# Xharlie/pointnerf

Hardware: AMD Instinct MI355X
Metric: rays/sec (render+bwd) NeRF-synth lego 800^2, K=8, 128 samp/ray (higher is better)
Workload: dtype f32 in / out / accumulate; forward GEMM operands as 2 x f16 planes (22-bit) on the f16 MFMA, 3 products per multiply-add; input-gradient GEMMs: f16 leading product + e4m3 cross terms (csrc/mixq.h), 2 product equivalents; weight-gradient GEMM operands as one f16 plane each

## Files before the change

### pointnerf_amd/csrc/backward.hip

```cpp
#include "mixq.h"

namespace {
constexpr int WG_CHUNKS = 256;
constexpr size_t PARTIAL_FLOATS = (size_t)WG_CHUNKS * PN_H * PN_IN1P;

struct BwdArgs {
    pnerf_camera cam;
    const float *params;
    const float4 *packed;
    const float *raydir;
    const int *pidx, *valid_list, *counters;
    const int *cls_list, *cls_info;
    int cls;
    int SR, K, TS;
    long long cap_samples;
    const float *decoded, *weight, *grad_decoded;
    PnSaved sv;
    const float *emb;
    float *gparams;
    float *g_emb, *g_conf, *g_dir, *g_color;
    const float *conf, *zo_gs;
    float zo_eps;
};
struct BwdXArgs : BwdArgs {
    const float *xyz, *sample_loc;
    float *g_xyz;
};
template <bool XYZG> struct BwdArgsOf { using T = BwdArgs; };
template <> struct BwdArgsOf<true> { using T = BwdXArgs; };

__global__ __launch_bounds__(256) void k_grad_max(const int *__restrict__ list, const int *__restrict__ counters, long long cap, const float *__restrict__ gd,
                                                  unsigned *__restrict__ gscale) {
    __shared__ unsigned red[4];
    const long long Ns = counters[0] < cap ? counters[0] : cap;
    float m = 0.f;
    for (long long vs = (long long)blockIdx.x * 256 + threadIdx.x; vs < Ns; vs += (long long)gridDim.x * 256) {
        const float4 g = *reinterpret_cast<const float4 *>(gd + (long long)list[vs] * 4);
        m = fmaxf(m, fmaxf(fmaxf(fabsf(g.x), fabsf(g.y)), fmaxf(fabsf(g.z), fabsf(g.w))));
    }
#pragma unroll
    for (int off = 32; off > 0; off >>= 1) m = fmaxf(m, __shfl_xor(m, off, 64));
    if ((threadIdx.x & 63) == 0) red[threadIdx.x >> 6] = __float_as_uint(m);
    __syncthreads();
    if (threadIdx.x == 0) {
        unsigned r = red[0];
        for (int i = 1; i < 4; ++i) r = red[i] > r ? red[i] : r;
        if (r != 0u && r < 0x7f800000u) atomicMax(gscale, r);
    }
}
__device__ __forceinline__ void pn_scale_from_bits(unsigned mb, float &S, float &invS) {
    const int e = (int)((mb >> 23) & 0xffu);
    int se = (e == 0 || e == 255) ? 127 : 127 + 4 - (e - 127);
    se = se < 2 ? 2 : (se > 252 ? 252 : se);
    S = __uint_as_float((unsigned)se << 23);
    invS = __uint_as_float((unsigned)(254 - se) << 23);
}
static_assert(PN_CTILE == PN_TILE, "one row-scale record layout for both tile kernels");
constexpr int PN_RSC_BYTES = PN_TILE * 16 + PN_TILE * 2;
__device__ __forceinline__ void pn_sample_scale(const float4 g, float S, float invS, float &Si, float &invSi) {
    const unsigned mb = __float_as_uint(fmaxf(fmaxf(fabsf(g.x), fabsf(g.y)), fmaxf(fabsf(g.z), fabsf(g.w))));
    Si = S; invSi = invS;
    if (mb >= 0x00800000u && mb < 0x7f800000u) {
        pn_scale_from_bits(mb, Si, invSi);
        if (Si < S) { Si = S; invSi = invS; }
    }
}
struct PnRowScale {
    float *p;
    __device__ __forceinline__ void set(int r, float Si, float invSi, float S, float w = 0.f) const {
        const float f = S * invSi;
        *reinterpret_cast<float4 *>(p + 4 * r) = make_float4(Si, invSi, f, w * Si);
        reinterpret_cast<_Float16 *>(p + 4 * PN_TILE)[r] = (_Float16)f;
    }
    __device__ __forceinline__ float S(int r) const { return p[4 * r]; }
    __device__ __forceinline__ float inv(int r) const { return p[4 * r + 1]; }
    __device__ __forceinline__ float to_call(int r) const { return p[4 * r + 2]; }
    __device__ __forceinline__ float wS(int r) const { return p[4 * r + 3]; }
    __device__ __forceinline__ const char *h8(int rg) const { return reinterpret_cast<const char *>(p + 4 * PN_TILE) + rg * 16; }
};
template <int NF, int XRS = PN_XRS>
__device__ __forceinline__ void pn_copy_out_kmajor_hs(const char *X, const PnRowScale &rs, uint4 *__restrict__ dst, long long rg0, int tid) {
    const int lane = tid & 63, wave = tid >> 6;
    const int blk = ((lane >> 2) & 3) * XRS + ((lane >> 4) * 16 + (lane & 3) * 4) * 2;
#pragma unroll
    for (int i = 0; i < 2; ++i) {
        const int rg = wave * 2 + i;
        const char *src = X + rg * 8 * XRS + blk;
        uint4 *d = dst + (rg0 + rg) * NF;
        const uint4 fq = *reinterpret_cast<const uint4 *>(rs.h8(rg));
        const pn_h4 flo = __builtin_bit_cast(pn_h4, make_uint2(fq.x, fq.y)), fhi = __builtin_bit_cast(pn_h4, make_uint2(fq.z, fq.w));
        uint2 lo[(NF + 63) / 64], hi[(NF + 63) / 64];
#pragma unroll
        for (int j = 0; j < (NF + 63) / 64; ++j) { lo[j] = pn_lds_read_tr16(src + j * 128); hi[j] = pn_lds_read_tr16(src + 4 * XRS + j * 128); }
#pragma unroll
        for (int j = 0; j < (NF + 63) / 64; ++j) {
            const int f = lane + 64 * j;
            if (f < NF) {
                const uint2 a = __builtin_bit_cast(uint2, __builtin_bit_cast(pn_h4, lo[j]) * flo), b = __builtin_bit_cast(uint2, __builtin_bit_cast(pn_h4, hi[j]) * fhi);
                pn_f4 t = {__uint_as_float(a.x), __uint_as_float(a.y), __uint_as_float(b.x), __uint_as_float(b.y)};
                PN_STREAM_STORE(t, reinterpret_cast<pn_f4 *>(d + f));
            }
        }
    }
}

constexpr int CB_XRS = 2 * PN_HC + 16, CB_XPL = PN_CTILE * CB_XRS, CB_XBYTES = 2 * CB_XPL;
constexpr int CB_DRAW = CB_XBYTES, CB_GACC = CB_DRAW + PN_CTILE * 4 * 4, CB_W4 = CB_GACC + 6 * PN_HC * 4, CB_RSC = CB_W4 + 3 * PN_HC * 4, CB_BYTES = CB_RSC + PN_RSC_BYTES;
static_assert(3 * CB_BYTES <= 160 * 1024, "three colour workgroups must fit the 160 KB LDS");

__device__ __forceinline__ void cb_epilogue(const f32x16 (&acc)[2][2], unsigned mw, char *X, int wave, int lane) {
#pragma unroll
    for (int rb = 0; rb < 2; ++rb)
#pragma unroll
        for (int g = 0; g < 4; ++g) {
            const int f0 = pn_d_feat(wave, g, lane), row = 32 * rb + (lane & 31), e = rb * 16 + g * 4;
            float v[4];
#pragma unroll
            for (int i = 0; i < 4; ++i) v[i] = acc[0][rb][4 * g + i] * ((int)(mw << (e + i)) < 0 ? 0.01f : 1.f);
            pn_x_store4<true, CB_XRS, CB_XPL>(X, row, f0, v[0], v[1], v[2], v[3]);
        }
}
__device__ __forceinline__ void cb_bias_sums(const char *X, const PnRowScale &rs, int tid, float *__restrict__ gsum) {
    const int c0 = 8 * (tid & 15), r0 = 4 * (tid >> 4);
    float gb[8] = {0.f, 0.f, 0.f, 0.f, 0.f, 0.f, 0.f, 0.f};
#pragma unroll
    for (int rr = 0; rr < 4; ++rr) {
        const uint4 h = *reinterpret_cast<const uint4 *>(X + (r0 + rr) * CB_XRS + c0 * 2);
        const uint4 m = *reinterpret_cast<const uint4 *>(X + CB_XPL + (r0 + rr) * CB_XRS + c0 * 2);
        const float f = rs.to_call(r0 + rr);
        gb[0] = pn_fma2_lo(h.x, m.x, f, gb[0]); gb[1] = pn_fma2_hi(h.x, m.x, f, gb[1]);
        gb[2] = pn_fma2_lo(h.y, m.y, f, gb[2]); gb[3] = pn_fma2_hi(h.y, m.y, f, gb[3]);
        gb[4] = pn_fma2_lo(h.z, m.z, f, gb[4]); gb[5] = pn_fma2_hi(h.z, m.z, f, gb[5]);
        gb[6] = pn_fma2_lo(h.w, m.w, f, gb[6]); gb[7] = pn_fma2_hi(h.w, m.w, f, gb[7]);
    }
#pragma unroll
    for (int i = 0; i < 8; ++i) atomicAdd(gsum + c0 + i, gb[i]);
}

template <bool WG2>
__global__ __launch_bounds__(256, 3) void k_color_backward(BwdArgs a) {
    extern __shared__ __attribute__((aligned(16))) char smem_cb[];
    char *X = smem_cb;
    float *draw = reinterpret_cast<float *>(smem_cb + CB_DRAW);
    const PnRowScale rs{reinterpret_cast<float *>(smem_cb + CB_RSC)};
    const int Ns = a.counters[0] < a.cap_samples ? a.counters[0] : (int)a.cap_samples;
    const float *P = a.params;
    const char *img = reinterpret_cast<const char *>(a.packed);
    float S, invS;
    pn_scale_from_bits(a.sv.gscale[0], S, invS);
    if (blockIdx.x == 0 && threadIdx.x == 0) a.sv.cls_info[PN_CI_CTILES] = (Ns + PN_CTILE - 1) / PN_CTILE;
    float *gacc = reinterpret_cast<float *>(smem_cb + CB_GACC);
    for (int i = threadIdx.x; i < 6 * PN_HC; i += 256) gacc[i] = 0.f;
    float gb4x = 0.f, gb4y = 0.f, gb4z = 0.f;
    auto row_sample = [&](long long t) -> long long {
        const long long vs = t * PN_CTILE + threadIdx.x;
        return (threadIdx.x < PN_CTILE && vs < Ns) ? (long long)a.valid_list[vs] : -1;
    };
    float po[3] = {0.f, 0.f, 0.f}, pg[3] = {0.f, 0.f, 0.f}, pgs = 0.f;
    auto row_values = [&](long long si) {
        if (si >= 0) {
            const float *o = a.decoded + si * 4, *g = a.grad_decoded + si * 4;
            po[0] = o[1]; po[1] = o[2]; po[2] = o[3]; pgs = g[0]; pg[0] = g[1]; pg[1] = g[2]; pg[2] = g[3];
        }
    };
    long long si_cur = row_sample(blockIdx.x);
    row_values(si_cur);
    float *w4s = reinterpret_cast<float *>(smem_cb + CB_W4);
    for (int i = threadIdx.x; i < 3 * PN_HC; i += 256) w4s[i] = P[PO_WC4 + i];

    f32x16 acc[2][2];
    for (long long tile = blockIdx.x; tile * PN_CTILE < Ns; tile += gridDim.x) {
        int tid = threadIdx.x;
        asm volatile("" : "+v"(tid));
        const int lane = tid & 63, wave = __builtin_amdgcn_readfirstlane(tid >> 6);
        const long long grow0 = tile * PN_CTILE;
        PN_LDS_BARRIER();
        if (tid < PN_CTILE) {
            float d0 = 0.f, d1 = 0.f, d2 = 0.f, Si = S, invSi = invS;
            if (si_cur >= 0) {
                pn_sample_scale(make_float4(pgs, pg[0], pg[1], pg[2]), S, invS, Si, invSi);
                const float s0 = (po[0] + 0.001f) / 1.002f, s1 = (po[1] + 0.001f) / 1.002f, s2 = (po[2] + 0.001f) / 1.002f;
                d0 = pg[0] * 1.002f * s0 * (1.f - s0); d1 = pg[1] * 1.002f * s1 * (1.f - s1); d2 = pg[2] * 1.002f * s2 * (1.f - s2);
            }
            *reinterpret_cast<float4 *>(draw + tid * 4) = make_float4(d0, d1, d2, Si);
            rs.set(tid, Si, invSi, S);
            gb4x += d0; gb4y += d1; gb4z += d2;
        }
        const long long si_next = row_sample(tile + gridDim.x);
        PN_LDS_BARRIER();
        {
            const int c4 = tid & 31, rg = tid >> 5;
            float4 c3v[8];
            float w4[3][4], gw4[3][4], gb3[4] = {0.f, 0.f, 0.f, 0.f};
#pragma unroll
            for (int k = 0; k < 3; ++k) {
                const float4 w = *reinterpret_cast<const float4 *>(w4s + k * PN_HC + 4 * c4);
                w4[k][0] = w.x; w4[k][1] = w.y; w4[k][2] = w.z; w4[k][3] = w.w;
#pragma unroll
                for (int i = 0; i < 4; ++i) gw4[k][i] = 0.f;
            }
#pragma unroll
            for (int rr = 0; rr < 8; ++rr) c3v[rr] = *reinterpret_cast<const float4 *>(a.sv.c3 + (grow0 + 8 * rg + rr) * PN_HC + 4 * c4);
#pragma unroll
            for (int rr = 0; rr < 8; ++rr) {
                const int row = 8 * rg + rr;
                const float4 d = *reinterpret_cast<const float4 *>(draw + row * 4);
                const float c[4] = {c3v[rr].x, c3v[rr].y, c3v[rr].z, c3v[rr].w};
                float u[4];
#pragma unroll
                for (int i = 0; i < 4; ++i) {
                    u[i] = (d.x * w4[0][i] + d.y * w4[1][i] + d.z * w4[2][i]) * pn_lrelu_grad(c[i]);
                    gw4[0][i] += d.x * c[i]; gw4[1][i] += d.y * c[i]; gw4[2][i] += d.z * c[i];
                    gb3[i] += u[i];
                }
                pn_x_store4<true, CB_XRS, CB_XPL>(X, row, 4 * c4, u[0] * d.w, u[1] * d.w, u[2] * d.w, u[3] * d.w);
            }
#pragma unroll
            for (int i = 0; i < 4; ++i) {
#pragma unroll
                for (int k = 0; k < 3; ++k) atomicAdd(gacc + k * PN_HC + 4 * c4 + i, gw4[k][i]);
                atomicAdd(gacc + 3 * PN_HC + 4 * c4 + i, gb3[i]);
            }
        }
        PnGemmW<8, 4, 1, 4, 3> WD3;
        WD3.prefetch(reinterpret_cast<const uint4 *>(img + PKH_DC3), wave, lane);
        PN_LDS_BARRIER();
        pn_copy_out_kmajor_hs<PN_HC, CB_XRS>(X, rs, a.sv.dc3k, tile * 8, tid);
        if (WG2) pn_copy_out_kmajor_hs<PN_HC, CB_XRS>(X + CB_XPL, rs, a.sv.dc3m, tile * 8, tid);
        const unsigned mw2 = a.sv.cmask[(tile * 2 + 1) * 256 + tid], mw1 = a.sv.cmask[(tile * 2 + 0) * 256 + tid];
        pn_acc_zero(acc);
        pn_gemm_f16x3_run<8, 4, 1, 4, 3, CB_XRS, CB_XPL>(X, WD3, lane, acc);
        row_values(si_next);
        si_cur = si_next;
        PN_LDS_BARRIER();
        cb_epilogue(acc, mw2, X, wave, lane);
        PnGemmW<8, 4, 1, 4, 3> WD2;
        WD2.prefetch(reinterpret_cast<const uint4 *>(img + PKH_DC2), wave, lane);
        PN_LDS_BARRIER();
        cb_bias_sums(X, rs, tid, gacc + 4 * PN_HC);
        pn_copy_out_kmajor_hs<PN_HC, CB_XRS>(X, rs, a.sv.dc2k, tile * 8, tid);
        if (WG2) pn_copy_out_kmajor_hs<PN_HC, CB_XRS>(X + CB_XPL, rs, a.sv.dc2m, tile * 8, tid);
        pn_acc_zero(acc);
        pn_gemm_f16x3_run<8, 4, 1, 4, 3, CB_XRS, CB_XPL>(X, WD2, lane, acc);
        PN_LDS_BARRIER();
        cb_epilogue(acc, mw1, X, wave, lane);
        PnGemmW<8, 8, 2, 1, 3> WD1;
        WD1.prefetch(reinterpret_cast<const uint4 *>(img + PKH_DC1), 2 * wave, lane);
        PN_LDS_BARRIER();
        cb_bias_sums(X, rs, tid, gacc + 5 * PN_HC);
        pn_copy_out_kmajor_hs<PN_HC, CB_XRS>(X, rs, a.sv.dc1k, tile * 8, tid);
        if (WG2) pn_copy_out_kmajor_hs<PN_HC, CB_XRS>(X + CB_XPL, rs, a.sv.dc1m, tile * 8, tid);
        pn_acc_zero(acc);
        pn_gemm_f16x3_run<8, 8, 2, 1, 3, CB_XRS, CB_XPL>(X, WD1, lane, acc);
#pragma unroll
        for (int fb = 0; fb < 2; ++fb)
#pragma unroll
            for (int rb = 0; rb < 2; ++rb) {
                const float ri = rs.inv(32 * rb + (lane & 31));
#pragma unroll
                for (int g = 0; g < 4; ++g) {
                    pn_f4 t = {acc[fb][rb][4 * g] * ri, acc[fb][rb][4 * g + 1] * ri, acc[fb][rb][4 * g + 2] * ri, acc[fb][rb][4 * g + 3] * ri};
                    PN_REG_STORE(t, reinterpret_cast<pn_f4 *>(a.sv.dfs + (grow0 + 32 * rb + (lane & 31)) * PN_H + pn_d_feat(2 * wave + fb, g, lane)));
                }
            }
    }
    PN_LDS_BARRIER();
    {
        const int tid = threadIdx.x;
        for (int i = tid; i < 3 * PN_HC; i += 256) atomicAdd(&a.gparams[PO_WC4 + i], gacc[i]);
        if (tid < PN_HC) {
            atomicAdd(&a.gparams[PO_BC3 + tid], gacc[3 * PN_HC + tid]);
            atomicAdd(&a.gparams[PO_BC2 + tid], gacc[4 * PN_HC + tid] * invS);
            atomicAdd(&a.gparams[PO_BC1 + tid], gacc[5 * PN_HC + tid] * invS);
        }
        if (tid < PN_CTILE) {
#pragma unroll
            for (int off = 32; off > 0; off >>= 1) { gb4x += __shfl_xor(gb4x, off, 64); gb4y += __shfl_xor(gb4y, off, 64); gb4z += __shfl_xor(gb4z, off, 64); }
            if (tid == 0) { atomicAdd(&a.gparams[PO_BC4], gb4x); atomicAdd(&a.gparams[PO_BC4 + 1], gb4y); atomicAdd(&a.gparams[PO_BC4 + 2], gb4z); }
        }
    }
}

constexpr int BL_ROW = PN_XBYTES, BL_RSC = BL_ROW + 10 * PN_TILE * 4, BL_W5 = BL_RSC + PN_RSC_BYTES, BL_BYTES = BL_W5 + PN_H * 4;
constexpr int LDDX = 228;
static_assert(2 * BL_BYTES <= 160 * 1024, "two backward workgroups must fit the 160 KB LDS");
static_assert(PN_TILE * LDDX * 4 <= PN_XBYTES, "d X0 tile");
constexpr int LDDX_X = 292, BL_GW = BL_BYTES, BL_BYTES_X = BL_GW + PN_TILE * 4;
static_assert(2 * BL_BYTES_X <= 160 * 1024, "two xyz_grad backward workgroups must fit the 160 KB LDS");
static_assert(PN_TILE * LDDX_X * 4 <= PN_XBYTES, "d X0 tile (xyz_grad)");

template <bool MIX = false>
__device__ __forceinline__ void b_epilogue(const f32x16 (&acc)[PN_NFB][2], const unsigned (&mask)[PN_NFB], char *X, int wave, int lane) {
#pragma unroll
    for (int fb = 0; fb < PN_NFB; ++fb) {
        const unsigned mw = mask[fb];
#pragma unroll
        for (int rb = 0; rb < 2; ++rb)
#pragma unroll
            for (int g = 0; g < 4; ++g) {
                float v[4];
#pragma unroll
                for (int i = 0; i < 4; ++i) {
                    const int e = (rb * 4 + g) * 4 + i;
                    v[i] = acc[fb][rb][4 * g + i] * ((int)(mw << e) < 0 ? 0.01f : 1.f);
                }
                if (MIX) pn_xq_store4(X, 32 * rb + (lane & 31), pn_d_feat(PN_NFB * wave + fb, g, lane), v[0], v[1], v[2], v[3]);
                else pn_x_store4<true>(X, 32 * rb + (lane & 31), pn_d_feat(PN_NFB * wave + fb, g, lane), v[0], v[1], v[2], v[3]);
            }
    }
}

#ifdef PN_EMU
#define PN_WAVE_LDS_SYNC() __syncthreads()
#else
#define PN_WAVE_LDS_SYNC() asm volatile("s_waitcnt lgkmcnt(0)" ::: "memory")
#endif

template <int KC, bool MIX = false, bool XG = false>
__device__ __forceinline__ void b_front(const BwdArgs &a, char *X, const float *w5s, const float *wrow, const float *wnrm, const float *dsg, const float *xrow,
                                        float *draw, const int *sidx, const int *prow, const float4 (&dfr)[4], const float *dfb0, const PnRowScale &rs, int tid,
                                        float (&gw5)[8], float &gb5t, unsigned kinv = 0u, float *gwf = nullptr) {
    const int lane = tid & 63, cg = tid & 31, r0 = 8 * (tid >> 5);
    const int j0 = KC == 0 ? pn_row_div(r0, kinv) : 0;
    float zo_conf = 0.f;
    if (a.zo_gs && (lane & 3) == 0) {
        const int rz = prow[r0 + ((lane >> 4) & 1) * 4 + ((lane >> 3) & 1) * 2 + ((lane >> 2) & 1)];
        if (rz >= 0) zo_conf = a.conf[rz];
    }
    auto df_of = [&](int j, float4 &ga, float4 &gb) {
        if (KC >= 4) { ga = dfr[2 * j]; gb = dfr[2 * j + 1]; }
        else { ga = *reinterpret_cast<const float4 *>(dfb0 + j * PN_H); gb = *reinterpret_cast<const float4 *>(dfb0 + j * PN_H + 4); }
    };
    float pd[8];
#pragma unroll
    for (int i = 0; i < 8; ++i) {
        const int r = r0 + i, j = KC == 0 ? pn_row_div(r, kinv) - j0 : i / (KC == 0 ? 1 : KC);
        const uint4 h = *reinterpret_cast<const uint4 *>(X + r * PN_XRS + cg * 16);
        const uint4 m = *reinterpret_cast<const uint4 *>(X + PN_XPLANE + r * PN_XRS + cg * 16);
        float4 ga, gb;
        df_of(j, ga, gb);
        float s = 0.f;
        s = pn_fma2_lo(h.x, m.x, ga.x, s); s = pn_fma2_hi(h.x, m.x, ga.y, s); s = pn_fma2_lo(h.y, m.y, ga.z, s); s = pn_fma2_hi(h.y, m.y, ga.w, s);
        s = pn_fma2_lo(h.z, m.z, gb.x, s); s = pn_fma2_hi(h.z, m.z, gb.y, s); s = pn_fma2_lo(h.w, m.w, gb.z, s); s = pn_fma2_hi(h.w, m.w, gb.w, s);
        pd[i] = s;
    }
    {
        const bool b4 = lane & 16, b3 = lane & 8, b2 = lane & 4;
#pragma unroll
        for (int j = 0; j < 4; ++j) { const float send = b4 ? pd[j] : pd[j + 4], keep = b4 ? pd[j + 4] : pd[j]; pd[j] = keep + __shfl_xor(send, 16, 64); }
#pragma unroll
        for (int j = 0; j < 2; ++j) { const float send = b3 ? pd[j] : pd[j + 2], keep = b3 ? pd[j + 2] : pd[j]; pd[j] = keep + __shfl_xor(send, 8, 64); }
        { const float send = b2 ? pd[0] : pd[1], keep = b2 ? pd[1] : pd[0]; pd[0] = keep + __shfl_xor(send, 4, 64); }
        pd[0] += __shfl_xor(pd[0], 2, 64);
        pd[0] += __shfl_xor(pd[0], 1, 64);
        const int r = r0 + ((lane >> 4) & 1) * 4 + ((lane >> 3) & 1) * 2 + ((lane >> 2) & 1);
        if ((lane & 3) == 0) {
// ... 324 lines not shown
                for (int rb = 0; rb < 2; ++rb)
#pragma unroll
                    for (int g = 0; g < 4; ++g)
                        *reinterpret_cast<float4 *>(dx + (32 * rb + (lane & 31)) * LDX + pn_d_feat(PN_NFB * wave + fb, g, lane)) =
                            make_float4(acc[fb][rb][4 * g], acc[fb][rb][4 * g + 1], acc[fb][rb][4 * g + 2], acc[fb][rb][4 * g + 3]);
            }
        if constexpr (XYZG) {
            if (wave == 3) {
#pragma unroll
                for (int fb = 0; fb < 2; ++fb)
#pragma unroll
                    for (int rb = 0; rb < 2; ++rb)
#pragma unroll
                        for (int g = 0; g < 4; ++g) {
                            const f32x16 &v = fb == 0 ? acc1[0][rb] : acx[0][rb];
                            *reinterpret_cast<float4 *>(dx + (32 * rb + (lane & 31)) * LDX + pn_d_feat(PN_MB_D1 + fb, g, lane)) =
                                make_float4(v[4 * g], v[4 * g + 1], v[4 * g + 2], v[4 * g + 3]);
                        }
            }
        }
        PN_LDS_BARRIER();
        PN_TR(pn_trace_bwd, 15);
        if (rp >= 0) {
            float *dr_ = dx + row * LDX;
            const float e[8] = {e0.x, e0.y, e0.z, e0.w, e1.x, e1.y, e1.z, e1.w};
            float go[PN_EPT];
            const float ri = rs.inv(row);
#pragma unroll
            for (int i = 0; i < PN_EPT; ++i) {
                const int dd = PN_EPT * q + i;
                float s[3], c[3];
                pn_pe_octaves<3>(e[i], s, c);
                float g = dr_[dd], fr = 1.f;
#pragma unroll
                for (int f = 0; f < 3; ++f) {
                    const float2 t = *reinterpret_cast<const float2 *>(dr_ + PN_F + dd * 6 + 2 * f);
                    g += fr * (t.x * c[f] - t.y * s[f]);
                    fr *= 2.f;
                }
                go[i] = g * ri;
            }
#pragma unroll
            for (int i = 0; i < PN_EPT; i += 4) *reinterpret_cast<float4 *>(dr_ + PN_EPT * q + i) = make_float4(go[i], go[i + 1], go[i + 2], go[i + 3]);
        }
        PN_WAVE_LDS_SYNC();
        const int r0w = (row & ~15) + (lane >> 5), col = lane & 31;
#pragma unroll
        for (int j = 0; j < 8; ++j) {
            const int r = r0w + 2 * j, p = prow[r];
            if (p >= 0) atomicAdd(&a.g_emb[(long long)p * PN_F + col], dx[r * LDX + col]);
        }
        if constexpr (XYZG) b_xyz_row(a, dx + row * LDX, gwf, wrow, wnrm, sidx, rp, row, q, K, kinv, rs.inv(row));
        PN_TR(pn_trace_bwd, 16);
    }
    if (tile_first >= tile_last) return;
    {
        const int cg = tid0 & 31, rs = tid0 >> 5;
        float *red = reinterpret_cast<float *>(smem_b);
        PN_LDS_BARRIER();
        if (tid0 < PN_NTHR) {
#pragma unroll
            for (int c = 0; c < 8; ++c) red[rs * PN_H + 8 * cg + c] = gw5[c];
            if (cg == 0) red[8 * PN_H + rs] = gb5t;
        }
        PN_LDS_BARRIER();
        if (tid0 >= PN_H) return;
        float t = 0.f;
#pragma unroll
        for (int r = 0; r < 8; ++r) t += red[r * PN_H + tid0];
        atomicAdd(&a.gparams[PO_W5 + tid0], t * invS);
        if (tid0 == 0) {
            float b = 0.f;
            for (int r = 0; r < 8; ++r) b += red[8 * PN_H + r];
            atomicAdd(&a.gparams[PO_B5], b * invS);
        }
    }
}

#ifdef PN_EMU
#define PN_WAIT_VMCNT(n) ((void)0)
#else
#define PN_WAIT_VMCNT(n) asm volatile("s_waitcnt vmcnt(%0)" ::"n"(n) : "memory")
#endif
#ifndef PN_WG_RS
#define PN_WG_RS 32
#endif
#ifndef PN_WG_NST
#define PN_WG_NST 4
#endif
template <int N> __device__ __forceinline__ void pn_wait_vm_stages(int stages) {
    if (stages >= 3) PN_WAIT_VMCNT(3 * N);
    else if (stages == 2) PN_WAIT_VMCNT(2 * N);
    else if (stages == 1) PN_WAIT_VMCNT(N);
    else PN_WAIT_VMCNT(0);
}
template <int NFB, int MF, int RS, int NST, bool TWO = false>
__global__ __launch_bounds__(512) void k_wgrad_f16(const uint4 *__restrict__ A, const uint4 *__restrict__ B,
                                                   const int *__restrict__ d_tiles, float *__restrict__ partial,
                                                   const uint4 *__restrict__ Am = nullptr, const uint4 *__restrict__ Bm = nullptr) {
    constexpr int RG = RS / 8;
    constexpr int AU = RG * MF, BU = RG * NFB;
    constexpr int HALF = AU + BU;
    constexpr int STAGE = TWO ? 2 * HALF : HALF;
    constexpr int NI = STAGE / 64, NIW = (NI + 7) / 8;
    static_assert((NST - 2) * NIW <= 63 && NST >= 3 && NST <= 5, "vmcnt is a 6-bit count");
    constexpr int MTW = MF / 64, NTW = NFB >= 256 ? 2 : 1;
    constexpr int NMAIN = 4 * NTW * 32;
    constexpr bool TAIL_B = NFB > NMAIN, TAIL_ONES = !TAIL_B && MF == 256;
    static_assert(STAGE % 64 == 0, "a stage is a whole number of 1 KB wave copies");
    extern __shared__ __attribute__((aligned(16))) uint4 smem_w[];
    const int tid = threadIdx.x, lane = tid & 63, wave = __builtin_amdgcn_readfirstlane(tid >> 6);
    const int wm = wave >> 2, wn = wave & 3;
    const long long stages = (long long)(*d_tiles) * (PN_TILE / RS);
    const int nst = stages > (long long)blockIdx.x ? (int)((stages - blockIdx.x + gridDim.x - 1) / gridDim.x) : 0;
    f32x16 acc[MTW][NTW], acct;
#pragma unroll
    for (int r = 0; r < 16; ++r) {
        acct[r] = 0.f;
#pragma unroll
        for (int i = 0; i < MTW; ++i)
#pragma unroll
            for (int j = 0; j < NTW; ++j) acc[i][j][r] = 0.f;
    }
    auto issue = [&](int s, int buf) {
        const long long rg = (long long)RG * ((long long)blockIdx.x + (long long)gridDim.x * s);
#pragma unroll
        for (int i = 0; i < NIW; ++i) {
            const bool pad = wave + 8 * i >= NI;
            const int j = pad ? 0 : wave + 8 * i, u0 = 64 * j;
            const uint4 *dst = smem_w + (pad ? NST * STAGE : buf * STAGE + u0);
            const uint4 *src;
            if (u0 < AU) src = A + rg * MF + u0;
            else if (u0 < HALF) src = B + rg * NFB + (u0 - AU);
            else if (u0 < HALF + AU) src = Am + rg * MF + (u0 - HALF);
            else src = Bm + rg * NFB + (u0 - HALF - AU);
            __builtin_amdgcn_global_load_lds(src + lane, (__attribute__((address_space(3))) void *)dst, 16, 0, 0);
        }
    };
    pn_h8 ones = {0, 0, 0, 0, 0, 0, 0, 0};
    if ((lane & 31) == 0) ones = pn_h8{1, 1, 1, 1, 1, 1, 1, 1};
    const bool has_tail = (TAIL_B || TAIL_ONES) && (MF == 256 || wn < 2);
    if (nst > 0) {
#pragma unroll
        for (int i = 0; i < NST - 1; ++i) if (nst > i) issue(i, i);
        for (int s = 0; s < nst; ++s) {
            pn_wait_vm_stages<NIW>(nst - 1 - s < NST - 2 ? nst - 1 - s : NST - 2);
            __builtin_amdgcn_s_barrier();
            if (s + NST - 1 < nst) issue(s + NST - 1, (s + NST - 1) % NST);
            const uint4 *st = smem_w + (s % NST) * STAGE;
#pragma unroll
            for (int kk = 0; kk < RS / 16; ++kk) {
                const uint4 *fa = st + (2 * kk + (lane >> 5)) * MF + (lane & 31);
                const uint4 *fb = st + AU + (2 * kk + (lane >> 5)) * NFB + (lane & 31);
                pn_h8 ah[MTW], bh[NTW], am[TWO ? MTW : 1], bm[TWO ? NTW : 1];
#pragma unroll
                for (int i = 0; i < MTW; ++i) ah[i] = __builtin_bit_cast(pn_h8, fa[(MTW * wm + i) * 32]);
#pragma unroll
                for (int i = 0; i < NTW; ++i) bh[i] = __builtin_bit_cast(pn_h8, fb[(NTW * wn + i) * 32]);
                if (TWO) {
#pragma unroll
                    for (int i = 0; i < MTW; ++i) am[i] = __builtin_bit_cast(pn_h8, fa[HALF + (MTW * wm + i) * 32]);
#pragma unroll
                    for (int i = 0; i < NTW; ++i) bm[i] = __builtin_bit_cast(pn_h8, fb[HALF + (NTW * wn + i) * 32]);
                }
#pragma unroll
                for (int i = 0; i < MTW; ++i)
#pragma unroll
                    for (int j = 0; j < NTW; ++j)
                        acc[i][j] = __builtin_amdgcn_mfma_f32_32x32x16_f16(ah[i], bh[j], acc[i][j], 0, 0, 0);
                if (TWO) {
#pragma unroll
                    for (int i = 0; i < MTW; ++i)
#pragma unroll
                        for (int j = 0; j < NTW; ++j)
                            acc[i][j] = __builtin_amdgcn_mfma_f32_32x32x16_f16(ah[i], bm[j], acc[i][j], 0, 0, 0);
#pragma unroll
                    for (int i = 0; i < MTW; ++i)
#pragma unroll
                        for (int j = 0; j < NTW; ++j)
                            acc[i][j] = __builtin_amdgcn_mfma_f32_32x32x16_f16(am[i], bh[j], acc[i][j], 0, 0, 0);
                }
                if (has_tail) {
                    pn_h8 tah, tam = ah[0];
                    if (MF == 256) tah = wn == 0 ? ah[0] : wn == 1 ? ah[1] : wn == 2 ? ah[MTW > 2 ? 2 : 0] : ah[MTW > 3 ? 3 : 0];
                    else tah = wn == 0 ? ah[0] : ah[MTW > 1 ? 1 : 0];
                    if (TWO) {
                        if (MF == 256) tam = wn == 0 ? am[0] : wn == 1 ? am[TWO && MTW > 1 ? 1 : 0] : wn == 2 ? am[TWO && MTW > 2 ? 2 : 0] : am[TWO && MTW > 3 ? 3 : 0];
                        else tam = wn == 0 ? am[0] : am[TWO && MTW > 1 ? 1 : 0];
                    }
                    if (TAIL_B) {
                        acct = __builtin_amdgcn_mfma_f32_32x32x16_f16(tah, __builtin_bit_cast(pn_h8, fb[NMAIN]), acct, 0, 0, 0);
                        if (TWO) {
                            acct = __builtin_amdgcn_mfma_f32_32x32x16_f16(tah, __builtin_bit_cast(pn_h8, fb[HALF + NMAIN]), acct, 0, 0, 0);
                            acct = __builtin_amdgcn_mfma_f32_32x32x16_f16(tam, __builtin_bit_cast(pn_h8, fb[NMAIN]), acct, 0, 0, 0);
                        }
                    } else {
                        acct = __builtin_amdgcn_mfma_f32_32x32x16_f16(tah, ones, acct, 0, 0, 0);
                        if (TWO) acct = __builtin_amdgcn_mfma_f32_32x32x16_f16(tam, ones, acct, 0, 0, 0);
                    }
                }
            }
        }
    }
    float *out = partial + (size_t)blockIdx.x * 256 * 288;
#pragma unroll
    for (int i = 0; i < MTW; ++i)
#pragma unroll
        for (int j = 0; j < NTW; ++j)
#pragma unroll
            for (int r = 0; r < 16; ++r) {
                const int m = (MTW * wm + i) * 32 + (r & 3) + 8 * (r >> 2) + 4 * (lane >> 5);
                out[(size_t)m * 288 + (NTW * wn + j) * 32 + (lane & 31)] = acc[i][j][r];
            }
    if (has_tail) {
#pragma unroll
        for (int r = 0; r < 16; ++r) {
            const int m = (MTW * wm + wn) * 32 + (r & 3) + 8 * (r >> 2) + 4 * (lane >> 5);
            out[(size_t)m * 288 + 256 + (lane & 31)] = acct[r];
        }
    }
}

__global__ __launch_bounds__(256) void k_wgrad_reduce_f16(const float *__restrict__ partial, int chunks, int Mreal, int Nreal, int bias_col, const unsigned *__restrict__ gscale,
                                                          float *__restrict__ grad, int dst_w, int ldc, int dst_b) {
    __shared__ float part[4][64];
    const int lane = threadIdx.x & 63, w = threadIdx.x >> 6;
    const int e = blockIdx.x * 64 + lane;
    const size_t stride = (size_t)256 * 288;
    float s = 0.f;
    if (e < Mreal * 288) {
#pragma unroll 8
        for (int c = w; c < chunks; c += 4) s += partial[c * stride + e];
    }
    part[w][lane] = s;
    __syncthreads();
    if (w == 0 && e < Mreal * 288) {
        float S, invS;
        pn_scale_from_bits(gscale[0], S, invS);
        const int m = e / 288, n = e - m * 288;
        const float v = ((part[0][lane] + part[1][lane]) + (part[2][lane] + part[3][lane])) * invS;
        if (n < Nreal) grad[dst_w + m * ldc + n] += v;
        else if (n == bias_col) grad[dst_b + m] += v;
    }
}

enum WgShape { WG_288x256, WG_256x256, WG_288x128, WG_128x128 };
struct WgLayer {
    WgShape shape;
    const uint4 *dy, *x, *dym, *xm;
    const int *d_tiles;
    long long rows_max;
    int dst_w, ldc, nreal, bias_col, dst_b;
};
template <int NFB, int MF, int RS, int NST, bool TWO>
int launch_wgrad_f16(const WgLayer &L, float *partial, const unsigned *gscale, float *grad, hipStream_t s) {
    int chunks = WG_CHUNKS;
    const long long tiles = L.rows_max / PN_TILE;
    if (tiles < chunks) chunks = (int)(tiles > 0 ? tiles : 1);
    if ((size_t)chunks * 256 * 288 > PARTIAL_FLOATS) return PNERF_E_WS;
    if (TWO && (!L.dym || !L.xm)) return PNERF_E_INVAL;
    constexpr size_t lds = ((size_t)NST * (TWO ? 2 : 1) * (RS / 8) * (MF + NFB) + 64) * 16;
    static_assert(lds <= 160 * 1024, "wgrad ring");
    if (hipFuncSetAttribute((const void *)k_wgrad_f16<NFB, MF, RS, NST, TWO>, hipFuncAttributeMaxDynamicSharedMemorySize, (int)lds) != hipSuccess) return PNERF_E_LAUNCH;
    { PnProfScope prof(PNK_WGRAD, s);
    hipLaunchKernelGGL((k_wgrad_f16<NFB, MF, RS, NST, TWO>), dim3(chunks), dim3(512), lds, s, L.dy, L.x, L.d_tiles, partial, L.dym, L.xm); }
    PnProfScope prof(PNK_WGRAD_REDUCE, s);
    hipLaunchKernelGGL(k_wgrad_reduce_f16, dim3(pn_cdiv((long long)MF * 288, 64)), dim3(256), 0, s, partial, chunks, MF, L.nreal, L.bias_col, gscale, grad, L.dst_w, L.ldc, L.dst_b);
    PN_CHECK_LAUNCH();
    return 0;
}
template <bool TWO>
int launch_wgrad_layer(const WgLayer &L, float *partial, const unsigned *gscale, float *grad, hipStream_t s) {
    constexpr int RS = TWO ? 16 : PN_WG_RS, NST = TWO ? 4 : PN_WG_NST;
    switch (L.shape) {
        case WG_288x256: return launch_wgrad_f16<PN_NF1, PN_H, RS, NST, TWO>(L, partial, gscale, grad, s);
        case WG_256x256: return launch_wgrad_f16<PN_H, PN_H, RS, NST, TWO>(L, partial, gscale, grad, s);
        case WG_288x128: return launch_wgrad_f16<PN_NF1, PN_HC, 16, 4, TWO>(L, partial, gscale, grad, s);
        default: return launch_wgrad_f16<PN_HC, PN_HC, 16, 4, TWO>(L, partial, gscale, grad, s);
    }
}


struct WgX0Args {
    const int4 *rmeta;
    const float *emb;
    const uint4 *x0t;
    int n_points;
};
#ifndef PN_WX_RS
#define PN_WX_RS 32
#endif
#ifndef PN_WX_D
#define PN_WX_D (PN_WX_RS == 32 ? 3 : 7)
#endif
constexpr int WX_RS = PN_WX_RS, WX_RG = WX_RS / 8;
constexpr int WX_AU = WX_RG * PN_H;
constexpr int WX_NB = 224;
constexpr int WX_BU = WX_RG * WX_NB;
constexpr int WX_TU = WX_RG * 64;
constexpr int WX_GU = WX_RS * 8;
constexpr int WX_NA = WX_AU / 512;
constexpr int WX_L = WX_NA + 2;
constexpr int WX_D = PN_WX_D;
constexpr int WX_NST = WX_D + 1, WX_RMD = 2 * WX_D + 2, WX_GD = WX_D + 1;
constexpr int WX_RM_SLOTS = WX_D + 2, WX_G_SLOTS = WX_D + 1;
static_assert(WX_L * (WX_D - 1) <= 63 && WX_D >= 2, "vmcnt is a 6-bit count");
static_assert(WX_RS == 16 || WX_RS == 32, "rows per stage");
constexpr int WX_OFF_T = WX_NST * WX_AU, WX_OFF_B = WX_OFF_T + WX_NST * WX_TU, WX_OFF_RM = WX_OFF_B + 2 * WX_BU,
              WX_OFF_G = WX_OFF_RM + WX_RM_SLOTS * WX_RS, WX_OFF_PAD = WX_OFF_G + WX_G_SLOTS * WX_GU, WX_UNITS = WX_OFF_PAD + 64;
static_assert(WX_UNITS * 16 <= 160 * 1024, "k_wgrad_x0 LDS");

__device__ __forceinline__ void wx_store_h16(char *buf, int rg, int f, int rlow, _Float16 v) {
    *reinterpret_cast<_Float16 *>(buf + ((rg * WX_NB + f) * 16) + rlow * 2) = v;
}

__global__ __launch_bounds__(512) void k_wgrad_x0(const uint4 *__restrict__ A, WgX0Args g, const int *__restrict__ d_tiles, float *__restrict__ partial) {
    constexpr int MF = PN_H, MTW = 4;
    extern __shared__ __attribute__((aligned(16))) uint4 smem_x[];
    const int tid = threadIdx.x, lane = tid & 63, wave = __builtin_amdgcn_readfirstlane(tid >> 6);
    const int wm = wave >> 2, wn = wave & 3;
    const long long stages = (long long)(*d_tiles) * (PN_TILE / WX_RS);
    const int nst = stages > (long long)blockIdx.x ? (int)((stages - blockIdx.x + gridDim.x - 1) / gridDim.x) : 0;
    auto stage_rg = [&](int s) { return (long long)WX_RG * ((long long)blockIdx.x + (long long)gridDim.x * s); };
    f32x16 acc[MTW][2], acct;
#pragma unroll
    for (int r = 0; r < 16; ++r) {
        acct[r] = 0.f;
#pragma unroll
        for (int i = 0; i < MTW; ++i) { acc[i][0][r] = 0.f; acc[i][1][r] = 0.f; }
    }
    char *lds = reinterpret_cast<char *>(smem_x);
    int p_gather = 0;
    auto issue_a = [&](int s) {
        const bool ok = s < nst;
#pragma unroll
        for (int i = 0; i < WX_NA; ++i) {
            const int piece = wave + 8 * i;
            const uint4 *src = A + (ok ? stage_rg(s) * MF + 64 * piece : 0) + lane;
            const uint4 *dst = smem_x + (ok ? (s % WX_NST) * WX_AU + 64 * piece : WX_OFF_PAD);
            __builtin_amdgcn_global_load_lds(src, (__attribute__((address_space(3))) void *)dst, 16, 0, 0);
        }
        const bool okt = ok && wave < WX_RG;
        const uint4 *src = g.x0t + (okt ? (stage_rg(s) + wave) * 64 : 0) + lane;
        const uint4 *dst = smem_x + (okt ? WX_OFF_T + (s % WX_NST) * WX_TU + wave * 64 : WX_OFF_PAD);
        __builtin_amdgcn_global_load_lds(src, (__attribute__((address_space(3))) void *)dst, 16, 0, 0);
    };
    auto issue_second = [&](int s_rm, int s_g) {
        if (wave == 0) {
            const bool ok = s_rm < nst;
            const int4 *src = g.rmeta + (ok ? stage_rg(s_rm) * 8 : 0) + (lane & (WX_RS - 1));
            const uint4 *dst = smem_x + (ok ? WX_OFF_RM + (s_rm % WX_RM_SLOTS) * WX_RS : WX_OFF_PAD);
            if (lane < WX_RS) __builtin_amdgcn_global_load_lds(src, (__attribute__((address_space(3))) void *)dst, 16, 0, 0);
        } else if (wave <= WX_RG) {
            const bool ok = s_g < nst;
            const int p = ok ? p_gather : 0;
            const float *src = g.emb + (long long)p * PN_F + (lane >> 3) * 4;
            const uint4 *dst = smem_x + (ok ? WX_OFF_G + (s_g % WX_G_SLOTS) * WX_GU + (wave - 1) * 64 : WX_OFF_PAD);
            __builtin_amdgcn_global_load_lds(src, (__attribute__((address_space(3))) void *)dst, 16, 0, 0);
        } else {
            __builtin_amdgcn_global_load_lds(A + lane, (__attribute__((address_space(3))) void *)(smem_x + WX_OFF_PAD), 16, 0, 0);
        }
    };
    auto next_point = [&](int s_g) {
        if (wave >= 1 && wave <= WX_RG && s_g < nst) {
            const int p = reinterpret_cast<const int4 *>(smem_x + WX_OFF_RM + (s_g % WX_RM_SLOTS) * WX_RS)[8 * (wave - 1) + (lane & 7)].y;
            p_gather = p < 0 ? 0 : (p >= g.n_points ? g.n_points - 1 : p);
        }
    };
    auto build_into = [&](char *buf, const char *slot) {
#pragma unroll
        for (int it = 0; it < WX_RS / 16; ++it) {
            const int item = tid + 512 * it, rg = item >> 8, d = (item >> 3) & 31, rlow = item & 7;
            const float e = __builtin_amdgcn_fmed3f(*reinterpret_cast<const float *>(slot + rg * 1024 + ((d >> 2) * 8 + rlow) * 16 + (d & 3) * 4), -65504.f, 65504.f);
            float sn[3], cs[3];
            pn_pe_octaves<3>(e, sn, cs);
            const int f = PN_F + d * 6;
            wx_store_h16(buf, rg, d, rlow, (_Float16)e);
#pragma unroll
            for (int o = 0; o < 3; ++o) { wx_store_h16(buf, rg, f + 2 * o, rlow, (_Float16)sn[o]); wx_store_h16(buf, rg, f + 2 * o + 1, rlow, (_Float16)cs[o]); }
        }
    };
    auto build = [&](int s) {
        build_into(lds + (size_t)(WX_OFF_B + (s & 1) * WX_BU) * 16, lds + (size_t)(WX_OFF_G + (s % WX_G_SLOTS) * WX_GU) * 16);
    };
    if (nst > 0) {
        if (wave == 0)
            for (int s = 0; s < WX_RM_SLOTS; ++s) issue_second(s, 0);
        PN_WAIT_VMCNT(0);
        __syncthreads();
        for (int s = 0; s < WX_D; ++s) issue_a(s);
        if (wave >= 1 && wave <= WX_RG)
            for (int s = 0; s < WX_GD; ++s) { next_point(s); issue_second(0, s); }
        PN_WAIT_VMCNT(0);
        __syncthreads();
        if (wave == 0)
            for (int s = WX_RM_SLOTS; s < WX_RMD; ++s) issue_second(s, 0);
        PN_WAIT_VMCNT(0);
        __syncthreads();
        build(0);
        next_point(WX_GD);
        const long long stride_a = (long long)WX_RG * gridDim.x * MF, stride_t = (long long)WX_RG * gridDim.x * 64, stride_rm = (long long)WX_RG * gridDim.x * 8;
        const uint4 *pa = A + stage_rg(WX_D) * MF + 64 * wave + lane;
        const uint4 *pt = g.x0t + (stage_rg(WX_D) + wave) * 64 + lane;
        const int4 *prm = g.rmeta + stage_rg(WX_RMD) * 8 + (lane & (WX_RS - 1));
        int ia = WX_D % WX_NST, ig = WX_GD % WX_G_SLOTS, irm = WX_RMD % WX_RM_SLOTS;
        int ra = 0, rgs = 1 % WX_G_SLOTS, rrm = (1 + WX_GD) % WX_RM_SLOTS;
        const int n_main = nst - WX_RMD > 0 ? nst - WX_RMD : 0;
        auto bump = [](int &c, int n) { c = c + 1 == n ? 0 : c + 1; };
        for (int s = 0; s < nst; ++s) {
            PN_WAIT_VMCNT(WX_L * (WX_D - 1));
            PN_LDS_BARRIER();
            if (s < n_main) {
#pragma unroll
                for (int i = 0; i < WX_NA; ++i)
                    __builtin_amdgcn_global_load_lds(pa + 512 * i, (__attribute__((address_space(3))) void *)(smem_x + ia * WX_AU + 64 * (wave + 8 * i)), 16, 0, 0);
                if (wave < WX_RG) __builtin_amdgcn_global_load_lds(pt, (__attribute__((address_space(3))) void *)(smem_x + WX_OFF_T + ia * WX_TU + wave * 64), 16, 0, 0);
                else __builtin_amdgcn_global_load_lds(A + lane, (__attribute__((address_space(3))) void *)(smem_x + WX_OFF_PAD), 16, 0, 0);
                if (wave == 0) {
                    if (lane < WX_RS) __builtin_amdgcn_global_load_lds(prm, (__attribute__((address_space(3))) void *)(smem_x + WX_OFF_RM + irm * WX_RS), 16, 0, 0);
                } else if (wave <= WX_RG) {
                    __builtin_amdgcn_global_load_lds(g.emb + (long long)p_gather * PN_F + (lane >> 3) * 4,
                                                     (__attribute__((address_space(3))) void *)(smem_x + WX_OFF_G + ig * WX_GU + (wave - 1) * 64), 16, 0, 0);
                } else {
                    __builtin_amdgcn_global_load_lds(A + lane, (__attribute__((address_space(3))) void *)(smem_x + WX_OFF_PAD), 16, 0, 0);
                }
            } else {
                issue_a(s + WX_D);
                issue_second(s + WX_RMD, s + WX_GD);
            }
            pa += stride_a; pt += stride_t; prm += stride_rm;
#pragma unroll
            for (int kk = 0; kk < WX_RS / 16; ++kk) {
                const uint4 *fa = smem_x + ra * WX_AU + (2 * kk + (lane >> 5)) * MF + (lane & 31);
                const uint4 *fb = smem_x + WX_OFF_B + (s & 1) * WX_BU + (2 * kk + (lane >> 5)) * WX_NB + (lane & 31);
                const uint4 *ft = smem_x + WX_OFF_T + ra * WX_TU + (2 * kk + (lane >> 5)) * 64 + (lane & 31);
                pn_h8 ah[MTW], bh[2];
#pragma unroll
                for (int i = 0; i < MTW; ++i) ah[i] = __builtin_bit_cast(pn_h8, fa[(MTW * wm + i) * 32]);
                const pn_h8 tah = __builtin_bit_cast(pn_h8, fa[(MTW * wm + wn) * 32]);
                bh[0] = __builtin_bit_cast(pn_h8, fb[(2 * wn) * 32]);
                bh[1] = __builtin_bit_cast(pn_h8, wn < 3 ? fb[(2 * wn + 1) * 32] : ft[0]);
#pragma unroll
                for (int i = 0; i < MTW; ++i)
#pragma unroll
                    for (int j = 0; j < 2; ++j)
                        acc[i][j] = __builtin_amdgcn_mfma_f32_32x32x16_f16(ah[i], bh[j], acc[i][j], 0, 0, 0);
                acct = __builtin_amdgcn_mfma_f32_32x32x16_f16(tah, __builtin_bit_cast(pn_h8, ft[32]), acct, 0, 0, 0);
            }
            build_into(lds + (size_t)(WX_OFF_B + ((s + 1) & 1) * WX_BU) * 16, lds + (size_t)(WX_OFF_G + rgs * WX_GU) * 16);
            if (wave >= 1 && wave <= WX_RG && s + 1 + WX_GD < nst) {
                const int p = reinterpret_cast<const int4 *>(smem_x + WX_OFF_RM + rrm * WX_RS)[8 * (wave - 1) + (lane & 7)].y;
                p_gather = p < 0 ? 0 : (p >= g.n_points ? g.n_points - 1 : p);
            }
            bump(ia, WX_NST); bump(ig, WX_G_SLOTS); bump(irm, WX_RM_SLOTS); bump(ra, WX_NST); bump(rgs, WX_G_SLOTS); bump(rrm, WX_RM_SLOTS);
        }
    }
    float *out = partial + (size_t)blockIdx.x * 256 * 288;
#pragma unroll
    for (int i = 0; i < MTW; ++i)
#pragma unroll
        for (int j = 0; j < 2; ++j)
#pragma unroll
            for (int r = 0; r < 16; ++r) {
                const int m = (MTW * wm + i) * 32 + (r & 3) + 8 * (r >> 2) + 4 * (lane >> 5);
                out[(size_t)m * 288 + (2 * wn + j) * 32 + (lane & 31)] = acc[i][j][r];
            }
#pragma unroll
    for (int r = 0; r < 16; ++r) {
        const int m = (MTW * wm + wn) * 32 + (r & 3) + 8 * (r >> 2) + 4 * (lane >> 5);
        out[(size_t)m * 288 + 256 + (lane & 31)] = acct[r];
    }
}

int launch_wgrad_x0(const uint4 *A, const WgX0Args &g, const int *d_tiles, long long rows_max, float *partial, const unsigned *gscale,
                    float *grad, hipStream_t s) {
    int chunks = WG_CHUNKS;
    const long long tiles = rows_max / PN_TILE;
    if (tiles < chunks) chunks = (int)(tiles > 0 ? tiles : 1);
    if ((size_t)chunks * 256 * 288 > PARTIAL_FLOATS) return PNERF_E_WS;
    constexpr size_t lds = (size_t)WX_UNITS * 16;
    if (hipFuncSetAttribute((const void *)k_wgrad_x0, hipFuncAttributeMaxDynamicSharedMemorySize, (int)lds) != hipSuccess) return PNERF_E_LAUNCH;
    { PnProfScope prof(PNK_WGRAD, s);
    hipLaunchKernelGGL(k_wgrad_x0, dim3(chunks), dim3(512), lds, s, A, g, d_tiles, partial); }
    PnProfScope prof(PNK_WGRAD_REDUCE, s);
    hipLaunchKernelGGL(k_wgrad_reduce_f16, dim3(pn_cdiv((long long)PN_H * 288, 64)), dim3(256), 0, s, partial, chunks, PN_H, PN_IN1, PN_ONES1, gscale, grad, (int)PO_W1, (int)PN_IN1, (int)PO_B1);
    PN_CHECK_LAUNCH();
    return 0;
}
}

size_t pn_wgrad_partials_bytes() { return pn_align(PARTIAL_FLOATS * sizeof(float)); }

namespace {
__global__ void k_zero_one_empty(const float *__restrict__ conf, const int *__restrict__ counters, long long slots_per_ray, const float *__restrict__ gs, float eps,
                                 float *__restrict__ g_conf) {
    const long long n_empty = (long long)counters[1] * slots_per_ray - (long long)counters[3];
    if (n_empty <= 0) return;
    const float g = PnZeroOne(conf[0], eps).grad(gs[0]);
    if (g != 0.f) atomicAdd(&g_conf[0], g * (float)n_empty);
// ... 84 lines not shown
```

Measured before the change: 2.079 million.

## Replace colour-backward LDS atomics with per-wave partial sums and tune wgrad loads

In the colour backward kernel, the LDS atomicAdd reductions are replaced by per-wave private gradient-sum slices, combined with a shuffle across half-waves followed by plain read-modify-write. The four slices are summed at the end before the global atomics. The c3 and cmask loads are hoisted to the top of each tile so their latency overlaps the barrier. Separately, the wgrad and x-grad global_load_lds calls now pass a nonzero aux (cache-policy) bit. The 128-wide wgrad layers get a configurable row-stage size and a chunk count based on rows per stage. The cost is more LDS per workgroup, which still has to fit three workgroups, and the cache-policy effect depends on the hardware.

```diff
diff --git a/pointnerf_amd/csrc/backward.hip b/pointnerf_amd/csrc/backward.hip
--- a/pointnerf_amd/csrc/backward.hip
+++ b/pointnerf_amd/csrc/backward.hip
@@ -105,7 +105,8 @@
 }
 
 constexpr int CB_XRS = 2 * PN_HC + 16, CB_XPL = PN_CTILE * CB_XRS, CB_XBYTES = 2 * CB_XPL;
-constexpr int CB_DRAW = CB_XBYTES, CB_GACC = CB_DRAW + PN_CTILE * 4 * 4, CB_W4 = CB_GACC + 6 * PN_HC * 4, CB_RSC = CB_W4 + 3 * PN_HC * 4, CB_BYTES = CB_RSC + PN_RSC_BYTES;
+constexpr int CB_GSUMS = 6 * PN_HC;
+constexpr int CB_DRAW = CB_XBYTES, CB_GACC = CB_DRAW + PN_CTILE * 4 * 4, CB_W4 = CB_GACC + 4 * CB_GSUMS * 4, CB_RSC = CB_W4 + 3 * PN_HC * 4, CB_BYTES = CB_RSC + PN_RSC_BYTES;
 static_assert(3 * CB_BYTES <= 160 * 1024, "three colour workgroups must fit the 160 KB LDS");
 
 __device__ __forceinline__ void cb_epilogue(const f32x16 (&acc)[2][2], unsigned mw, char *X, int wave, int lane) {
@@ -121,20 +122,24 @@
         }
 }
 __device__ __forceinline__ void cb_bias_sums(const char *X, const PnRowScale &rs, int tid, float *__restrict__ gsum) {
-    const int c0 = 8 * (tid & 15), r0 = 4 * (tid >> 4);
-    float gb[8] = {0.f, 0.f, 0.f, 0.f, 0.f, 0.f, 0.f, 0.f};
-#pragma unroll
-    for (int rr = 0; rr < 4; ++rr) {
-        const uint4 h = *reinterpret_cast<const uint4 *>(X + (r0 + rr) * CB_XRS + c0 * 2);
-        const uint4 m = *reinterpret_cast<const uint4 *>(X + CB_XPL + (r0 + rr) * CB_XRS + c0 * 2);
+    const int cp = tid & 63, r0 = 16 * (tid >> 6);
+    float g0 = 0.f, g1 = 0.f;
+#pragma unroll
+    for (int rr = 0; rr < 16; ++rr) {
+        const unsigned h = *reinterpret_cast<const unsigned *>(X + (r0 + rr) * CB_XRS + cp * 4);
+        const unsigned m = *reinterpret_cast<const unsigned *>(X + CB_XPL + (r0 + rr) * CB_XRS + cp * 4);
         const float f = rs.to_call(r0 + rr);
-        gb[0] = pn_fma2_lo(h.x, m.x, f, gb[0]); gb[1] = pn_fma2_hi(h.x, m.x, f, gb[1]);
-        gb[2] = pn_fma2_lo(h.y, m.y, f, gb[2]); gb[3] = pn_fma2_hi(h.y, m.y, f, gb[3]);
-        gb[4] = pn_fma2_lo(h.z, m.z, f, gb[4]); gb[5] = pn_fma2_hi(h.z, m.z, f, gb[5]);
-        gb[6] = pn_fma2_lo(h.w, m.w, f, gb[6]); gb[7] = pn_fma2_hi(h.w, m.w, f, gb[7]);
-    }
-#pragma unroll
-    for (int i = 0; i < 8; ++i) atomicAdd(gsum + c0 + i, gb[i]);
+        g0 = pn_fma2_lo(h, m, f, g0); g1 = pn_fma2_hi(h, m, f, g1);
+    }
+    float2 *d = reinterpret_cast<float2 *>(gsum) + cp;
+    const float2 t = *d;
+    *d = make_float2(t.x + g0, t.y + g1);
+}
+
+__device__ __forceinline__ void cb_add4(float *__restrict__ d, const float (&v)[4]) {
+    float4 *p = reinterpret_cast<float4 *>(d);
+    const float4 t = *p;
+    *p = make_float4(t.x + v[0], t.y + v[1], t.z + v[2], t.w + v[3]);
 }
 
 template <bool WG2>
@@ -150,7 +155,8 @@
     pn_scale_from_bits(a.sv.gscale[0], S, invS);
     if (blockIdx.x == 0 && threadIdx.x == 0) a.sv.cls_info[PN_CI_CTILES] = (Ns + PN_CTILE - 1) / PN_CTILE;
     float *gacc = reinterpret_cast<float *>(smem_cb + CB_GACC);
-    for (int i = threadIdx.x; i < 6 * PN_HC; i += 256) gacc[i] = 0.f;
+    for (int i = threadIdx.x; i < 4 * CB_GSUMS; i += 256) gacc[i] = 0.f;
+    float *gaccw = gacc + (threadIdx.x >> 6) * CB_GSUMS;
     float gb4x = 0.f, gb4y = 0.f, gb4z = 0.f;
     auto row_sample = [&](long long t) -> long long {
         const long long vs = t * PN_CTILE + threadIdx.x;
@@ -174,6 +180,10 @@
         asm volatile("" : "+v"(tid));
         const int lane = tid & 63, wave = __builtin_amdgcn_readfirstlane(tid >> 6);
         const long long grow0 = tile * PN_CTILE;
+        float4 c3v[8];
+#pragma unroll
+        for (int rr = 0; rr < 8; ++rr) c3v[rr] = *reinterpret_cast<const float4 *>(a.sv.c3 + (grow0 + 8 * (tid >> 5) + rr) * PN_HC + 4 * (tid & 31));
+        const unsigned mw2 = a.sv.cmask[(tile * 2 + 1) * 256 + tid], mw1 = a.sv.cmask[(tile * 2 + 0) * 256 + tid];
         PN_LDS_BARRIER();
         if (tid < PN_CTILE) {
             float d0 = 0.f, d1 = 0.f, d2 = 0.f, Si = S, invSi = invS;
@@ -190,7 +200,6 @@
         PN_LDS_BARRIER();
         {
             const int c4 = tid & 31, rg = tid >> 5;
-            float4 c3v[8];
             float w4[3][4], gw4[3][4], gb3[4] = {0.f, 0.f, 0.f, 0.f};
 #pragma unroll
             for (int k = 0; k < 3; ++k) {
@@ -199,8 +208,6 @@
 #pragma unroll
                 for (int i = 0; i < 4; ++i) gw4[k][i] = 0.f;
             }
-#pragma unroll
-            for (int rr = 0; rr < 8; ++rr) c3v[rr] = *reinterpret_cast<const float4 *>(a.sv.c3 + (grow0 + 8 * rg + rr) * PN_HC + 4 * c4);
 #pragma unroll
             for (int rr = 0; rr < 8; ++rr) {
                 const int row = 8 * rg + rr;
@@ -218,8 +225,13 @@
 #pragma unroll
             for (int i = 0; i < 4; ++i) {
 #pragma unroll
-                for (int k = 0; k < 3; ++k) atomicAdd(gacc + k * PN_HC + 4 * c4 + i, gw4[k][i]);
-                atomicAdd(gacc + 3 * PN_HC + 4 * c4 + i, gb3[i]);
+                for (int k = 0; k < 3; ++k) gw4[k][i] += __shfl_xor(gw4[k][i], 32, 64);
+                gb3[i] += __shfl_xor(gb3[i], 32, 64);
+            }
+            if (lane < 32) {
+#pragma unroll
+                for (int k = 0; k < 3; ++k) cb_add4(gaccw + k * PN_HC + 4 * c4, gw4[k]);
+                cb_add4(gaccw + 3 * PN_HC + 4 * c4, gb3);
             }
         }
         PnGemmW<8, 4, 1, 4, 3> WD3;
@@ -227,7 +239,6 @@
         PN_LDS_BARRIER();
         pn_copy_out_kmajor_hs<PN_HC, CB_XRS>(X, rs, a.sv.dc3k, tile * 8, tid);
         if (WG2) pn_copy_out_kmajor_hs<PN_HC, CB_XRS>(X + CB_XPL, rs, a.sv.dc3m, tile * 8, tid);
-        const unsigned mw2 = a.sv.cmask[(tile * 2 + 1) * 256 + tid], mw1 = a.sv.cmask[(tile * 2 + 0) * 256 + tid];
         pn_acc_zero(acc);
         pn_gemm_f16x3_run<8, 4, 1, 4, 3, CB_XRS, CB_XPL>(X, WD3, lane, acc);
         row_values(si_next);
@@ -237,7 +248,7 @@
         PnGemmW<8, 4, 1, 4, 3> WD2;
         WD2.prefetch(reinterpret_cast<const uint4 *>(img + PKH_DC2), wave, lane);
         PN_LDS_BARRIER();
-        cb_bias_sums(X, rs, tid, gacc + 4 * PN_HC);
+        cb_bias_sums(X, rs, tid, gaccw + 4 * PN_HC);
         pn_copy_out_kmajor_hs<PN_HC, CB_XRS>(X, rs, a.sv.dc2k, tile * 8, tid);
         if (WG2) pn_copy_out_kmajor_hs<PN_HC, CB_XRS>(X + CB_XPL, rs, a.sv.dc2m, tile * 8, tid);
         pn_acc_zero(acc);
@@ -247,7 +258,7 @@
         PnGemmW<8, 8, 2, 1, 3> WD1;
         WD1.prefetch(reinterpret_cast<const uint4 *>(img + PKH_DC1), 2 * wave, lane);
         PN_LDS_BARRIER();
-        cb_bias_sums(X, rs, tid, gacc + 5 * PN_HC);
+        cb_bias_sums(X, rs, tid, gaccw + 5 * PN_HC);
         pn_copy_out_kmajor_hs<PN_HC, CB_XRS>(X, rs, a.sv.dc1k, tile * 8, tid);
         if (WG2) pn_copy_out_kmajor_hs<PN_HC, CB_XRS>(X + CB_XPL, rs, a.sv.dc1m, tile * 8, tid);
         pn_acc_zero(acc);
@@ -267,11 +278,12 @@
     PN_LDS_BARRIER();
     {
         const int tid = threadIdx.x;
-        for (int i = tid; i < 3 * PN_HC; i += 256) atomicAdd(&a.gparams[PO_WC4 + i], gacc[i]);
+        auto total = [&](int i) { return (gacc[i] + gacc[CB_GSUMS + i]) + (gacc[2 * CB_GSUMS + i] + gacc[3 * CB_GSUMS + i]); };
+        for (int i = tid; i < 3 * PN_HC; i += 256) atomicAdd(&a.gparams[PO_WC4 + i], total(i));
         if (tid < PN_HC) {
-            atomicAdd(&a.gparams[PO_BC3 + tid], gacc[3 * PN_HC + tid]);
-            atomicAdd(&a.gparams[PO_BC2 + tid], gacc[4 * PN_HC + tid] * invS);
-            atomicAdd(&a.gparams[PO_BC1 + tid], gacc[5 * PN_HC + tid] * invS);
+            atomicAdd(&a.gparams[PO_BC3 + tid], total(3 * PN_HC + tid));
+            atomicAdd(&a.gparams[PO_BC2 + tid], total(4 * PN_HC + tid) * invS);
+            atomicAdd(&a.gparams[PO_BC1 + tid], total(5 * PN_HC + tid) * invS);
         }
         if (tid < PN_CTILE) {
 #pragma unroll
@@ -762,11 +774,20 @@
 #else
 #define PN_WAIT_VMCNT(n) asm volatile("s_waitcnt vmcnt(%0)" ::"n"(n) : "memory")
 #endif
+#ifndef PN_WG_AUX
+#define PN_WG_AUX 2
+#endif
+#ifndef PN_WX_AUX
+#define PN_WX_AUX 2
+#endif
 #ifndef PN_WG_RS
 #define PN_WG_RS 32
 #endif
 #ifndef PN_WG_NST
 #define PN_WG_NST 4
+#endif
+#ifndef PN_WGC_RS
+#define PN_WGC_RS 32
 #endif
 template <int N> __device__ __forceinline__ void pn_wait_vm_stages(int stages) {
     if (stages >= 3) PN_WAIT_VMCNT(3 * N);
@@ -814,7 +835,7 @@
             else if (u0 < HALF) src = B + rg * NFB + (u0 - AU);
             else if (u0 < HALF + AU) src = Am + rg * MF + (u0 - HALF);
             else src = Bm + rg * NFB + (u0 - HALF - AU);
-            __builtin_amdgcn_global_load_lds(src + lane, (__attribute__((address_space(3))) void *)dst, 16, 0, 0);
+            __builtin_amdgcn_global_load_lds(src + lane, (__attribute__((address_space(3))) void *)dst, 16, 0, PN_WG_AUX);
         }
     };
     pn_h8 ones = {0, 0, 0, 0, 0, 0, 0, 0};
@@ -935,8 +956,8 @@
 template <int NFB, int MF, int RS, int NST, bool TWO>
 int launch_wgrad_f16(const WgLayer &L, float *partial, const unsigned *gscale, float *grad, hipStream_t s) {
     int chunks = WG_CHUNKS;
-    const long long tiles = L.rows_max / PN_TILE;
-    if (tiles < chunks) chunks = (int)(tiles > 0 ? tiles : 1);
+    const long long most = MF == PN_HC ? L.rows_max / ((long long)RS * NST) : L.rows_max / PN_TILE;
+    if (most < chunks) chunks = (int)(most > 0 ? most : 1);
     if ((size_t)chunks * 256 * 288 > PARTIAL_FLOATS) return PNERF_E_WS;
     if (TWO && (!L.dym || !L.xm)) return PNERF_E_INVAL;
     constexpr size_t lds = ((size_t)NST * (TWO ? 2 : 1) * (RS / 8) * (MF + NFB) + 64) * 16;
@@ -951,12 +972,12 @@
 }
 template <bool TWO>
 int launch_wgrad_layer(const WgLayer &L, float *partial, const unsigned *gscale, float *grad, hipStream_t s) {
-    constexpr int RS = TWO ? 16 : PN_WG_RS, NST = TWO ? 4 : PN_WG_NST;
+    constexpr int RS = TWO ? 16 : PN_WG_RS, NST = TWO ? 4 : PN_WG_NST, RSC = TWO ? 16 : PN_WGC_RS;
     switch (L.shape) {
         case WG_288x256: return launch_wgrad_f16<PN_NF1, PN_H, RS, NST, TWO>(L, partial, gscale, grad, s);
         case WG_256x256: return launch_wgrad_f16<PN_H, PN_H, RS, NST, TWO>(L, partial, gscale, grad, s);
-        case WG_288x128: return launch_wgrad_f16<PN_NF1, PN_HC, 16, 4, TWO>(L, partial, gscale, grad, s);
-        default: return launch_wgrad_f16<PN_HC, PN_HC, 16, 4, TWO>(L, partial, gscale, grad, s);
+        case WG_288x128: return launch_wgrad_f16<PN_NF1, PN_HC, RSC, 4, TWO>(L, partial, gscale, grad, s);
+        default: return launch_wgrad_f16<PN_HC, PN_HC, RSC, 4, TWO>(L, partial, gscale, grad, s);
     }
 }
 
@@ -1018,12 +1039,12 @@
             const int piece = wave + 8 * i;
             const uint4 *src = A + (ok ? stage_rg(s) * MF + 64 * piece : 0) + lane;
             const uint4 *dst = smem_x + (ok ? (s % WX_NST) * WX_AU + 64 * piece : WX_OFF_PAD);
-            __builtin_amdgcn_global_load_lds(src, (__attribute__((address_space(3))) void *)dst, 16, 0, 0);
+            __builtin_amdgcn_global_load_lds(src, (__attribute__((address_space(3))) void *)dst, 16, 0, PN_WX_AUX);
         }
         const bool okt = ok && wave < WX_RG;
         const uint4 *src = g.x0t + (okt ? (stage_rg(s) + wave) * 64 : 0) + lane;
         const uint4 *dst = smem_x + (okt ? WX_OFF_T + (s % WX_NST) * WX_TU + wave * 64 : WX_OFF_PAD);
-        __builtin_amdgcn_global_load_lds(src, (__attribute__((address_space(3))) void *)dst, 16, 0, 0);
+        __builtin_amdgcn_global_load_lds(src, (__attribute__((address_space(3))) void *)dst, 16, 0, PN_WX_AUX);
     };
     auto issue_second = [&](int s_rm, int s_g) {
         if (wave == 0) {
@@ -1093,8 +1114,8 @@
             if (s < n_main) {
 #pragma unroll
                 for (int i = 0; i < WX_NA; ++i)
-                    __builtin_amdgcn_global_load_lds(pa + 512 * i, (__attribute__((address_space(3))) void *)(smem_x + ia * WX_AU + 64 * (wave + 8 * i)), 16, 0, 0);
-                if (wave < WX_RG) __builtin_amdgcn_global_load_lds(pt, (__attribute__((address_space(3))) void *)(smem_x + WX_OFF_T + ia * WX_TU + wave * 64), 16, 0, 0);
+                    __builtin_amdgcn_global_load_lds(pa + 512 * i, (__attribute__((address_space(3))) void *)(smem_x + ia * WX_AU + 64 * (wave + 8 * i)), 16, 0, PN_WX_AUX);
+                if (wave < WX_RG) __builtin_amdgcn_global_load_lds(pt, (__attribute__((address_space(3))) void *)(smem_x + WX_OFF_T + ia * WX_TU + wave * 64), 16, 0, PN_WX_AUX);
                 else __builtin_amdgcn_global_load_lds(A + lane, (__attribute__((address_space(3))) void *)(smem_x + WX_OFF_PAD), 16, 0, 0);
                 if (wave == 0) {
                     if (lane < WX_RS) __builtin_amdgcn_global_load_lds(prm, (__attribute__((address_space(3))) void *)(smem_x + WX_OFF_RM + irm * WX_RS), 16, 0, 0);
```

New measurement: 2.115 million, median of 6. 1.8% higher.
